# HuiGuanLab/Lite-MKD

Measured on AMD Instinct MI355X. Metric: episodes/sec (5-way 5-shot, 8x224^2 frames), higher is better.
Workload: dtype f32

## Files before the change

### lite-mkd_amd/csrc/conv.hip

```cpp
#include "gemm_core.h"
#include <atomic>
#include <mutex>

struct ConvGemmArgs {
  const float* src;
  const float* wpk;
  float* out;
  float* stat_partial;
  int N, Hs, Ws, Cs;
  int Hr, Wr, rows_per_class, tiles_per_class;
  int sh;
  int Ho, Wo, Co, omul;
  int Kp, cps, nclass;
  int n_rt, n_ct, xcd_mode;
  int taps_pm1;
  int grid_step;
  int grid_total;
  int same;
  int halo;
  int accum;
  const float* ep_stats;
  const float* ep_res;
  int ep_relu;
  const float* pre_stats;
// ... 1115 lines not shown
  return p.tiles_per_class;
}
extern "C" int lmkd_conv2d_fwd_row_tiles(int N, int H, int W, int Cout, int KH, int KW, int stride, int pad) {
  return lmkd_conv2d_fwd_row_tiles_cs(N, H, W, 32, Cout, KH, KW, stride, pad);
}

static int conv2d_fwd_impl(const float* x, const float* wp, float* y, float* stat_partial, const float* ep_stats,
                           const float* ep_res, int ep_relu, int N, int H, int W, int Cs, int Cout, int KH, int KW, int stride,
                           int pad, void* stream, const float* pre_stats = nullptr, int seg_n0 = 0, const lmkd_amax_desc* am = nullptr) {
  LMKD_REQUIRE(x && wp && y, "lmkd_conv2d_fwd: null pointer");
  if (seg_n0 <= 0 || seg_n0 >= N) seg_n0 = 0;
  LMKD_REQUIRE(!seg_n0 || (conv_planes() && !ep_stats), "lmkd_conv2d_fwd_seg: two frame segments exist in the bf16-plane modes (training / plain forward)");
  LMKD_REQUIRE(aligned16(x) && aligned16(wp), "lmkd_conv2d_fwd: x / packed weights must be 16-byte aligned");
  LMKD_REQUIRE(Cs % 32 == 0 || Cs == 4, "lmkd_conv2d_fwd: channel count %d must be 4 (padded stem) or a multiple of 32", Cs);
  LMKD_REQUIRE(N > 0 && H > 0 && W > 0 && Cout > 0, "lmkd_conv2d_fwd: empty tensor");
  const bool smallc = Cs == 4;
  const int KWp = kw_padded(Cs, KW);
  LMKD_REQUIRE(!smallc || KWp == 8, "lmkd_conv2d_fwd: padded-stem path needs KW <= 8");
  LMKD_REQUIRE(KH * (smallc ? 1 : KW) <= LMKD_MAX_TAPS, "lmkd_conv2d_fwd: kernel %dx%d has too many taps", KH, KW);
  LMKD_REQUIRE(H < 32768 && W < 32768, "lmkd_conv2d_fwd: spatial dims too large");
  const bool act16 = g_lmkd_act_bf16;
  LMKD_REQUIRE(!pre_stats || (stat_partial && !smallc && !act16),
               "lmkd_conv2d_fwd_pre: the fused BatchNorm+ReLU loader exists for the training forward with fp32 activations (stat_partial given, Cs %% 32 == 0)");
  LMKD_REQUIRE(!act16 || (conv_nprod() == 1 && !ep_stats), "bf16 activations need lmkd_conv_set_compute_dtype(1) (training / plain forward)");
  const int Ho = conv_out(H, KH, stride, pad), Wo = conv_out(W, KW, stride, pad);
  LMKD_REQUIRE(Ho > 0 && Wo > 0, "lmkd_conv2d_fwd: empty output");
  LMKD_REQUIRE((long)N * H * W * Cs < 2147483647L && (long)N * Ho * Wo * Cout < 2147483647L,
               "lmkd_conv2d_fwd: tensor exceeds 2^31 elements");
  LMKD_REQUIRE(!conv_planes() || (long)N * H * W * Cs * (act16 && Cs != 4 ? 2 : 4) < 0xffffffe0L,
               "lmkd_conv2d_fwd: input tensor exceeds the 4 GiB buffer range of the bf16-plane kernels");
  ConvGemmArgs a;
  fwd_geometry(a, N, H, W, Cs, Cout, KH, KW, stride, pad, seg_n0);
  a.src = x; a.wpk = wp; a.out = y; a.stat_partial = stat_partial;
  a.h2_xw = am ? (const unsigned*)am->x_words : nullptr;
  a.amax_out = am ? (unsigned*)am->out_words : nullptr;
  note_fenced(am);
  a.ep_stats = ep_stats; a.ep_res = ep_res; a.ep_relu = ep_relu;
  a.pre_stats = pre_stats;
  const ConvPlan p = plan_fwd(a, KH, KW, pad);
  if (p.src2) {
    LMKD_REQUIRE((long)N * H * W * Cs * 4 < 2147483647L, "lmkd_conv2d_fwd: input tensor exceeds the 2 GiB offset range of the stride-2 patch form");
    fwd_src2_args(a, W, KWp);
  }
  int rc = launch_conv(a, p, (hipStream_t)stream);
  if (rc == LMKD_OK && a.amax_out && p.amax_pass) {
    const long per = (long)Ho * Wo * Cout, n0 = seg_n0 ? seg_n0 * per : (long)N * per;
    rc = amax_impl(y, n0, a.amax_out, stream, false);
    if (rc == LMKD_OK && seg_n0) rc = amax_impl(y + n0, (long)N * per - n0, a.amax_out + LMKD_AMAX_SEG_WORDS, stream, false);
  }
  return rc;
}

extern "C" int lmkd_conv2d_fwd(const float* x, const float* wp, float* y, float* stat_partial, int N, int H, int W, int Cs,
                               int Cout, int KH, int KW, int stride, int pad, void* stream) {
  return conv2d_fwd_impl(x, wp, y, stat_partial, nullptr, nullptr, 0, N, H, W, Cs, Cout, KH, KW, stride, pad, stream);
}

extern "C" int lmkd_conv2d_fwd_seg(const float* x, const float* pre_stats, const float* wp, float* y, float* stat_partial, int N, int H, int W,
                                   int Cs, int Cout, int KH, int KW, int stride, int pad, int seg_n0, void* stream, const lmkd_amax_desc* amax) {
  return conv2d_fwd_impl(x, wp, y, stat_partial, nullptr, nullptr, 0, N, H, W, Cs, Cout, KH, KW, stride, pad, stream, pre_stats, seg_n0, amax);
}

extern "C" int lmkd_conv2d_fwd_pre(const float* x_raw, const float* pre_stats, const float* wp, float* y, float* stat_partial, int N,
                                   int H, int W, int Cs, int Cout, int KH, int KW, int stride, int pad, void* stream) {
  LMKD_REQUIRE(pre_stats, "lmkd_conv2d_fwd_pre: BatchNorm table of the input missing");
  return conv2d_fwd_impl(x_raw, wp, y, stat_partial, nullptr, nullptr, 0, N, H, W, Cs, Cout, KH, KW, stride, pad, stream, pre_stats);
}

extern "C" int lmkd_conv2d_fwd_bn(const float* x, const float* wp, float* y, const float* bn_stats, const float* res, int relu,
                                  int N, int H, int W, int Cs, int Cout, int KH, int KW, int stride, int pad, void* stream, const lmkd_amax_desc* amax) {
  LMKD_REQUIRE(bn_stats, "lmkd_conv2d_fwd_bn: BatchNorm table missing");
  LMKD_REQUIRE(!g_lmkd_act_bf16, "lmkd_conv2d_fwd_bn: fp32 tensors only (with bf16 tensors run lmkd_conv2d_fwd + lmkd_bn_apply)");
  LMKD_REQUIRE(!conv_planes() || Cs % 32 == 0, "lmkd_conv2d_fwd_bn: the bf16-plane modes need Cs %% 32 == 0 (Cs=%d)", Cs);
  return conv2d_fwd_impl(x, wp, y, nullptr, bn_stats, res, relu, N, H, W, Cs, Cout, KH, KW, stride, pad, stream, nullptr, 0, amax);
}

static int bwd_data_args(ConvGemmArgs& a, const float* dy, const float* wd, float* dx, int N, int H, int W, int Cin, int Cout, int KH, int KW,
                         int stride, int pad, int accumulate, int seg_n0 = 0, const lmkd_amax_desc* am = nullptr) {
  if (seg_n0 <= 0 || seg_n0 >= N) seg_n0 = 0;
  LMKD_REQUIRE(!seg_n0 || conv_planes(), "lmkd_conv2d_bwd_data_seg: two frame segments exist in the bf16-plane modes");
  LMKD_REQUIRE(Cout % 32 == 0, "lmkd_conv2d_bwd_data: Cout=%d must be a multiple of 32", Cout);
  LMKD_REQUIRE(stride == 1 || stride == 2, "lmkd_conv2d_bwd_data: stride %d unsupported", stride);
  LMKD_REQUIRE(KH * KW <= LMKD_MAX_TAPS, "lmkd_conv2d_bwd_data: kernel too large");
  LMKD_REQUIRE(!g_lmkd_act_bf16 || conv_nprod() == 1, "bf16 activations need lmkd_conv_set_compute_dtype(1)");
  const int Ho = conv_out(H, KH, stride, pad), Wo = conv_out(W, KW, stride, pad);
  LMKD_REQUIRE((long)N * H * W * Cin < 2147483647L && (long)N * Ho * Wo * Cout < 2147483647L,
               "lmkd_conv2d_bwd_data: tensor exceeds 2^31 elements");
  LMKD_REQUIRE(!conv_planes() || (long)N * Ho * Wo * Cout * (g_lmkd_act_bf16 ? 2 : 4) < 0xffffffe0L,
               "lmkd_conv2d_bwd_data: dy exceeds the 4 GiB buffer range of the bf16-plane kernels");
  dgrad_geometry(a, N, H, W, Cin, Cout, KH, KW, stride, pad, seg_n0);
  a.src = dy; a.wpk = wd; a.out = dx; a.accum = accumulate;
  a.h2_xw = am ? (const unsigned*)am->dy_words : nullptr;
  return LMKD_OK;
}

extern "C" int lmkd_conv2d_bwd_data(const float* dy, const float* wd, float* dx, int N, int H, int W, int Cin, int Cout,
                                    int KH, int KW, int stride, int pad, int accumulate, void* stream) {
  LMKD_REQUIRE(dy && wd && dx, "lmkd_conv2d_bwd_data: null pointer");
  LMKD_REQUIRE(aligned16(dy) && aligned16(wd), "lmkd_conv2d_bwd_data: operands must be 16-byte aligned");
  ConvGemmArgs a;
  if (const int rc = bwd_data_args(a, dy, wd, dx, N, H, W, Cin, Cout, KH, KW, stride, pad, accumulate)) return rc;
  return launch_conv(a, plan_dgrad(a), (hipStream_t)stream);
}

extern "C" int lmkd_conv2d_bwd_data_bn_tiles_seg(int N, int H, int W, int Cin, int Cout, int KH, int KW, int stride, int pad, int seg_n0, int* tiles0) {
  if (stride != 1 || Cout % 32 != 0 || KH * KW > LMKD_MAX_TAPS) return 0;
  ConvGemmArgs a;
  if (bwd_data_args(a, nullptr, nullptr, nullptr, N, H, W, Cin, Cout, KH, KW, stride, pad, 0, seg_n0)) return 0;
  const ConvPlan p = plan_dgrad(a);
  if (!p.bnb_form) return 0;
  if (tiles0) *tiles0 = p.seg_t0;
  return p.tiles_per_class;
}
extern "C" int lmkd_conv2d_bwd_data_bn_tiles(int N, int H, int W, int Cin, int Cout, int KH, int KW, int stride, int pad) {
  return lmkd_conv2d_bwd_data_bn_tiles_seg(N, H, W, Cin, Cout, KH, KW, stride, pad, 0, nullptr);
}
extern "C" int lmkd_conv2d_bwd_data_seg(const float* dy, const float* wd, float* dx, const float* bn_x, const float* bn_stats, float* part, int N,
                                        int H, int W, int Cin, int Cout, int KH, int KW, int stride, int pad, int accumulate, int seg_n0, void* stream,
                                        const lmkd_amax_desc* amax) {
  LMKD_REQUIRE(dy && wd && dx, "lmkd_conv2d_bwd_data_seg: null pointer");
  LMKD_REQUIRE(aligned16(dy) && aligned16(wd), "lmkd_conv2d_bwd_data_seg: operands must be 16-byte aligned");
  LMKD_REQUIRE((bn_x != nullptr) == (bn_stats != nullptr) && (bn_x != nullptr) == (part != nullptr), "lmkd_conv2d_bwd_data_seg: bn_x, bn_stats and part go together");
  ConvGemmArgs a;
  if (const int rc = bwd_data_args(a, dy, wd, dx, N, H, W, Cin, Cout, KH, KW, stride, pad, accumulate, seg_n0, amax)) return rc;
  note_fenced(amax);
  if (bn_x) {
    LMKD_REQUIRE(!accumulate && aligned16(bn_x) && aligned16(bn_stats), "lmkd_conv2d_bwd_data_seg: the fused BatchNorm sums need a plain (non-accumulating) launch and aligned operands");
    a.bnb_x = bn_x; a.bnb_stats = bn_stats; a.stat_partial = part;
  }
  const ConvPlan p = plan_dgrad(a);
  LMKD_REQUIRE(!bn_x || p.bnb_form, "lmkd_conv2d_bwd_data_seg: this launch has no fused form (lmkd_conv2d_bwd_data_bn_tiles_seg returned 0)");
  return launch_conv(a, p, (hipStream_t)stream);
}
extern "C" int lmkd_conv2d_bwd_data_bn(const float* dy, const float* wd, float* dx, const float* bn_x, const float* bn_stats, float* part,
                                       int N, int H, int W, int Cin, int Cout, int KH, int KW, int stride, int pad, void* stream) {
  LMKD_REQUIRE(dy && wd && dx && bn_x && bn_stats && part, "lmkd_conv2d_bwd_data_bn: null pointer");
  LMKD_REQUIRE(aligned16(dy) && aligned16(wd) && aligned16(bn_x) && aligned16(bn_stats), "lmkd_conv2d_bwd_data_bn: operands must be 16-byte aligned");
  ConvGemmArgs a;
  if (const int rc = bwd_data_args(a, dy, wd, dx, N, H, W, Cin, Cout, KH, KW, stride, pad, 0)) return rc;
  a.bnb_x = bn_x; a.bnb_stats = bn_stats; a.stat_partial = part;
  const ConvPlan p = plan_dgrad(a);
  LMKD_REQUIRE(p.bnb_form, "lmkd_conv2d_bwd_data_bn: this launch has no fused form (lmkd_conv2d_bwd_data_bn_tiles returned 0)");
  return launch_conv(a, p, (hipStream_t)stream);
}

static int g_wgrad_planes = 1;
extern "C" int lmkd_conv_set_wgrad_planes(int on) { g_wgrad_planes = on ? 1 : 0; return LMKD_OK; }
static int g_wgrad_win16 = 1;
extern "C" int lmkd_conv_set_wgrad_win16(int on) { g_wgrad_win16 = on ? 1 : 0; return LMKD_OK; }
static int g_wgrad_window = 1;
extern "C" int lmkd_conv_set_wgrad_window(int on) { g_wgrad_window = on < 0 ? 0 : on; return LMKD_OK; }
static inline bool wgrad_win_eligible(int W, int Cs, int Cout, int KH, int KW, int stride, int pad) {
  return g_wgrad_window && g_wgrad_planes && conv_planes() && KH == 3 && KW == 3 && stride == 1 && pad == 1 &&
         Cs % 32 == 0 && 32 + 2 * (W + 1) <= 256;
}
static void wgrad_win_plan(int Mpix, int W, int Cs, int Cout, int* cob, int* splits, int* steps_per_split) {
  *cob = Cout >= 128 ? 4 : 2;
  const int tiles = cdiv(Cout, 32 * *cob) * (Cs / 32);
  const int steps = cdiv(Mpix, LMKD_BK);
  const int warm = cdiv(2 * (W + 1), LMKD_BK);
  const int resident = 256 * ((conv_nprod() >= 6 && *cob == 2) ? 2 : 8 / *cob);
  int sp = g_wgrad_window > 1 ? cdiv(g_wgrad_window, tiles)
                              : std::max((int)(((long)resident * steps + 19600L * 4 / *cob) / (39200L * 4 / *cob)), cdiv(128, tiles));
  const int cap = std::max(1, steps / (12 * warm));
  if (sp > cap) sp = cap;
  *steps_per_split = cdiv(steps, sp);
  *splits = cdiv(steps, *steps_per_split);
}

static void wgrad_plan(int Mpix, int Cout, int Kp, int* splits, int* steps_per_split, int* bm, int* bn, bool planes = false) {
  *bm = Cout <= 64 ? 64 : 128;
  *bn = (Kp % 128 == 0 && Kp >= 1024) ? 128 : 64;
  int per_cu = (*bm == 128 && *bn == 128) ? 2 : ((*bm == 64 && *bn == 64) ? 4 : 3);
  if (planes) {
    if (*bm == 64 && *bn == 128) *bn = 64;
    const int npl = conv_nprod() == 1 ? 1 : 3;
    const long lds = 1L * npl * LMKD_BK * ((*bm * 2 + 64) + (*bn * 2 + 64));
    per_cu = (int)(160 * 1024 / lds);
    if (per_cu > 4) per_cu = 4;
    if (per_cu < 1) per_cu = 1;
  }
  const int tiles = cdiv(Cout, *bm) * cdiv(Kp, *bn);
  const int steps = cdiv(Mpix, LMKD_BK);
  const int slots = 256 * per_cu;
  int best_sp = 1;
  double best_cost = 1e30;
  for (int r = 1; r <= 3; ++r) {
    int sp = (slots * r) / tiles;
    if (sp > steps / 4) sp = steps / 4;
    if (sp < 1) sp = 1;
    const int sps = cdiv(steps, sp);
    sp = cdiv(steps, sps);
    const double rounds = (double)cdiv((long)tiles * sp, slots);
    const double cost = rounds * sps + 1.0 * sp / 8.0;
    if (cost < best_cost) { best_cost = cost; best_sp = sp; }
  }
  if (planes && *bm == 64 && *bn == 64 && best_sp < cdiv(steps, 64)) best_sp = cdiv(steps, 64);
  *steps_per_split = cdiv(steps, best_sp);
  *splits = cdiv(steps, *steps_per_split);
}

static int g_wgrad_stem = 1;
extern "C" int lmkd_conv_set_wgrad_stem(int on) { g_wgrad_stem = on ? 1 : 0; return LMKD_OK; }
static int stem_wgrad_plan(int N, int H, int W, int Cs, int Cout, int KH, int KW, int stride, int pad, int* G) {
  if (!g_wgrad_stem || !g_wgrad_planes || conv_nprod(g_lmkd_act_bf16) < 6 || Cs != 4 || Cout != 64 || KH != 7 || KW != 7 || stride != 2 || pad != 3) return 0;
  const int Ho = conv_out(H, KH, stride, pad), Wo = conv_out(W, KW, stride, pad);
  if (Wo < 17 || Wo > 128 || W > 2 * Wo || Ho < 1) return 0;
  const int units = N * cdiv(Ho, 2);
  int g = std::max(1, 2048 / (2 * Wo));
  g = std::min(g, std::max(1, units / 256));
  *G = g;
  return cdiv(units, g);
}

enum class WgFam : unsigned char {
  Stem,
  Win16,
  Win,
  Planes,
  Tile,
};
struct WgradPlan {
  WgFam fam;
  bool pre, act16, smallc;
  int nprod;
  int bm, bn;
  int cob;
  int G;
  int splits, splits0, sps0, sps1, seg_pix0;
  int xcd;
  int grid;
  long need;
  long ws;
};

static long wgrad_workspace(int N, int H, int W, int Cs, int Cout, int KH, int KW, int stride, int pad) {
  const int Ho = conv_out(H, KH, stride, pad), Wo = conv_out(W, KW, stride, pad);
  const int Kp = KH * kw_padded(Cs, KW) * Cs;
  int G, splits, sps, bm, bn;
  if (const int slabs = stem_wgrad_plan(N, H, W, Cs, Cout, KH, KW, stride, pad, &G)) return (long)slabs * Cout * Kp * sizeof(float);
  wgrad_plan(N * Ho * Wo, Cout, Kp, &splits, &sps, &bm, &bn, conv_planes() && g_wgrad_planes);
  if (wgrad_win_eligible(W, Cs, Cout, KH, KW, stride, pad)) {
    int cob, wsplits, wsps;
    wgrad_win_plan(N * Ho * Wo, W, Cs, Cout, &cob, &wsplits, &wsps);
    splits = std::max(splits, wsplits);
  }
  return (long)splits * Cout * Kp * sizeof(float);
}

static WgradPlan plan_wgrad(int N, int H, int W, int Cs, int Cout, int KH, int KW, int stride, int pad, int seg_n0, bool pre, bool maxima) {
  WgradPlan p;
  memset(&p, 0, sizeof(p));
  const bool act16 = g_lmkd_act_bf16;
  const int Ho = conv_out(H, KH, stride, pad), Wo = conv_out(W, KW, stride, pad);
  const int Kp = KH * kw_padded(Cs, KW) * Cs, Mpix = N * Ho * Wo;
  p.pre = pre; p.act16 = act16; p.smallc = Cs == 4;
  p.ws = wgrad_workspace(N, H, W, Cs, Cout, KH, KW, stride, pad);
  if (seg_n0)
    p.ws = std::max(p.ws, wgrad_workspace(seg_n0, H, W, Cs, Cout, KH, KW, stride, pad) + wgrad_workspace(N - seg_n0, H, W, Cs, Cout, KH, KW, stride, pad));
  p.seg_pix0 = seg_n0 ? seg_n0 * Ho * Wo : Mpix;
  if (const int slabs = stem_wgrad_plan(N, H, W, Cs, Cout, KH, KW, stride, pad, &p.G)) {
    p.fam = WgFam::Stem;
    p.nprod = conv_nprod(false, maxima);
    p.splits = p.grid = slabs;
  } else if (wgrad_win_eligible(W, Cs, Cout, KH, KW, stride, pad)) {
    const bool w16 = g_wgrad_win16 && conv_nprod(act16) >= 6;
    p.fam = w16 ? WgFam::Win16 : WgFam::Win;
    p.nprod = w16 ? conv_nprod(false, maxima) : conv_nprod(act16);
    wgrad_win_plan(Mpix, W, Cs, Cout, &p.cob, &p.splits, &p.sps0);
    p.splits0 = p.splits;
    if (seg_n0) {
      int sp1, cob1;
      wgrad_win_plan(p.seg_pix0, W, Cs, Cout, &p.cob, &p.splits0, &p.sps0);
      wgrad_win_plan(Mpix - p.seg_pix0, W, Cs, Cout, &cob1, &sp1, &p.sps1);
      p.splits = p.splits0 + sp1;
    }
    p.grid = 8 * cdiv(p.splits, 8) * cdiv(Cout, 32 * p.cob) * (Cs / 32);
  } else {
    const bool planes = conv_planes() && g_wgrad_planes;
    p.fam = planes ? WgFam::Planes : WgFam::Tile;
    p.nprod = planes ? conv_nprod(act16, maxima && !p.smallc && !pre) : (conv_nprod() == 1 ? 1 : 0);
    wgrad_plan(Mpix, Cout, Kp, &p.splits, &p.sps0, &p.bm, &p.bn, planes);
    p.splits0 = p.splits;
    if (seg_n0) {
      int sp1, bm1, bn1;
      wgrad_plan(p.seg_pix0, Cout, Kp, &p.splits0, &p.sps0, &p.bm, &p.bn, planes);
      wgrad_plan(Mpix - p.seg_pix0, Cout, Kp, &sp1, &p.sps1, &bm1, &bn1, planes);
      p.splits = p.splits0 + sp1;
    }
    p.xcd = (g_xcd_mode != 0 && g_xcd_mode != 1 && p.splits >= 32) ? 1 : 0;
    p.grid = (p.xcd ? 8 * cdiv(p.splits, 8) : p.splits) * cdiv(Cout, p.bm) * cdiv(Kp, p.bn);
  }
  p.need = (long)p.splits * Cout * Kp * sizeof(float);
  return p;
}

template <int NPROD, int D, int RLC>
static void launch_stem_wgrad(const StemWgradArgs& w, dim3 grid, size_t lds, hipStream_t s) {
  lds_attr_once<stem_wgrad_kernel<NPROD, D, RLC>>(160 * 1024);
  hipLaunchKernelGGL((stem_wgrad_kernel<NPROD, D, RLC>), grid, dim3(512), lds, s, w);
}
template <int NPROD>
static void launch_stem_wgrad(const StemWgradArgs& w, dim3 grid, size_t lds, hipStream_t s) {
  const bool deep = cdiv(2 * w.Wo, 32) >= 6;
  if (deep && w.RL == 1856) launch_stem_wgrad<NPROD, 6, 1856>(w, grid, lds, s);
  else if (deep) launch_stem_wgrad<NPROD, 6, 0>(w, grid, lds, s);
  else launch_stem_wgrad<NPROD, 2, 0>(w, grid, lds, s);
}
template <int COB>
static void launch_wgrad_win(const WgradWinArgs& w, const WgradPlan& p, bool big, hipStream_t s) {
  const dim3 grid(p.grid);
  if (p.fam == WgFam::Win16) {
    constexpr int JW = COB == 2 ? 1 : 2;
    constexpr int NT = 64 * COB * (2 / JW);
    with_nprod<3, 6, 9>(p.nprod, [&](auto np) {
      if (big && p.pre) hipLaunchKernelGGL((conv_wgrad_win16_kernel<COB, np, 256, true, 9, JW>), grid, dim3(NT), 0, s, w);
      else if (big) hipLaunchKernelGGL((conv_wgrad_win16_kernel<COB, np, 256, false, 9, JW>), grid, dim3(NT), 0, s, w);
      else if (p.pre) hipLaunchKernelGGL((conv_wgrad_win16_kernel<COB, np, 128, true, 9, JW>), grid, dim3(NT), 0, s, w);
      else hipLaunchKernelGGL((conv_wgrad_win16_kernel<COB, np, 128, false, 9, JW>), grid, dim3(NT), 0, s, w);
    });
    return;
  }
  auto go = [&](auto np, auto a16, auto pre) {
    constexpr int NPROD = decltype(np)::value;
    constexpr bool A16 = decltype(a16)::value, PRE = decltype(pre)::value;
    constexpr int TPW = (COB == 2 && NPROD != 1) ? 5 : 9;
    constexpr int NT = 64 * COB * ((9 + TPW - 1) / TPW);
    if (big) hipLaunchKernelGGL((conv_wgrad_win_kernel<COB, NPROD, A16, 256, PRE, TPW>), grid, dim3(NT), 0, s, w);
    else hipLaunchKernelGGL((conv_wgrad_win_kernel<COB, NPROD, A16, 128, PRE, TPW>), grid, dim3(NT), 0, s, w);
  };
  using T = std::true_type;
  using F = std::false_type;
  if (p.act16) go(std::integral_constant<int, 1>{}, T{}, F{});
  else with_nprod<1, 6, 9>(p.nprod, [&](auto np) { if (p.pre) go(np, F{}, T{}); else go(np, F{}, F{}); });
}

template <class CFG>
static void launch_wgrad_planes(const WgradArgs& a, const WgradPlan& p, hipStream_t s) {
  const dim3 grid(p.grid), block(256);
  if (p.act16) {
    if (p.smallc) hipLaunchKernelGGL((conv_wgrad_x3_kernel<CFG, true, 1, false, true>), grid, block, 0, s, a);
    else hipLaunchKernelGGL((conv_wgrad_x3_kernel<CFG, false, 1, false, true>), grid, block, 0, s, a);
  } else if (p.smallc) {
    with_nprod<1, 6, 9>(p.nprod, [&](auto np) { hipLaunchKernelGGL((conv_wgrad_x3_kernel<CFG, true, np, false>), grid, block, 0, s, a); });
  } else if (p.pre) {
    with_nprod<1, 6, 9>(p.nprod, [&](auto np) { hipLaunchKernelGGL((conv_wgrad_x3_kernel<CFG, false, np, true>), grid, block, 0, s, a); });
  } else {
    with_nprod<1, 3, 6, 9>(p.nprod, [&](auto np) { hipLaunchKernelGGL((conv_wgrad_x3_kernel<CFG, false, np, false>), grid, block, 0, s, a); });
  }
}

template <class CFG, bool SM, int THR>
static void launch_wgrad_tile(const WgradArgs& a, const WgradPlan& p, hipStream_t s) {
  const dim3 grid(p.grid);
  if (p.nprod == 1) hipLaunchKernelGGL((conv_wgrad_kernel<CFG, SM, true>), grid, dim3(THR), 0, s, a);
  else if (!SM && p.pre) hipLaunchKernelGGL((conv_wgrad_kernel<CFG, false, false, true>), grid, dim3(THR), 0, s, a);
  else hipLaunchKernelGGL((conv_wgrad_kernel<CFG, SM, false>), grid, dim3(THR), 0, s, a);
}

static int conv2d_bwd_weight_impl(const float* x, const float* pre_stats, const float* dy, float* dw_oihw, float* workspace,
                                  long ws_bytes, int N, int H, int W, int Cs, int Cin, int Cout, int KH, int KW, int stride, int pad,
                                  void* stream, int accumulate = 0, int seg_n0 = 0, const lmkd_amax_desc* am = nullptr) {
  const unsigned* amax_x = am ? (const unsigned*)am->x_words : nullptr;
  const unsigned* amax_dy = am ? (const unsigned*)am->dy_words : nullptr;
  note_fenced(am);
  LMKD_REQUIRE(x && dy && dw_oihw && workspace, "lmkd_conv2d_bwd_weight: null pointer");
  if (seg_n0 <= 0 || seg_n0 >= N) seg_n0 = 0;
  LMKD_REQUIRE(aligned16(x) && aligned16(dy) && aligned16(workspace), "lmkd_conv2d_bwd_weight: operands must be 16-byte aligned");
  LMKD_REQUIRE(Cs % 32 == 0 || Cs == 4, "lmkd_conv2d_bwd_weight: channel count %d must be 4 or a multiple of 32", Cs);
  LMKD_REQUIRE(Cout % 4 == 0, "lmkd_conv2d_bwd_weight: Cout %% 4 != 0");
  const bool smallc = Cs == 4;
  const WgradPlan p = plan_wgrad(N, H, W, Cs, Cout, KH, KW, stride, pad, seg_n0, pre_stats != nullptr, amax_x && amax_dy);
  LMKD_REQUIRE(!seg_n0 || p.fam != WgFam::Tile, "lmkd_conv2d_bwd_weight_seg: two frame segments exist in the bf16-plane modes");
  LMKD_REQUIRE(!pre_stats || (!smallc && (conv_nprod() != 1 || p.fam != WgFam::Tile) && !p.act16), "lmkd_conv2d_bwd_weight_pre: Cs %% 32 == 0, fp32 activations only");
  LMKD_REQUIRE(!p.act16 || (conv_nprod() == 1 && p.fam != WgFam::Tile), "bf16 activations need lmkd_conv_set_compute_dtype(1) and the plane weight-gradient kernel");
  const int Ho = conv_out(H, KH, stride, pad), Wo = conv_out(W, KW, stride, pad);
  const int KWp = kw_padded(Cs, KW), Kp = KH * KWp * Cs, Mpix = N * Ho * Wo;
  LMKD_REQUIRE((long)N * H * W * Cs < 2147483647L && (long)Mpix * Cout < 2147483647L, "lmkd_conv2d_bwd_weight: tensor too large");
  LMKD_REQUIRE(ws_bytes >= p.need, "lmkd_conv2d_bwd_weight: workspace too small");
  hipStream_t s = (hipStream_t)stream;
  if (p.fam == WgFam::Stem) {
    LMKD_REQUIRE((long)Mpix * 64 * 4 < 0xffffffe0L && (long)N * H * W * 16 < 0xffffffe0L, "lmkd_conv2d_bwd_weight: tensor too large for 32-bit byte offsets");
    StemWgradArgs w;
    memset(&w, 0, sizeof(w));
    w.dy = dy; w.x = x; w.slab = workspace;
    w.h2_xw = amax_x; w.h2_dyw = amax_dy;
    w.N = N; w.H = H; w.W = W; w.Ho = Ho; w.Wo = Wo;
    w.upi = cdiv(Ho, 2); w.units = N * w.upi; w.G = p.G; w.slabs = p.splits;
    w.RL = 16 * Wo + 64;
    const size_t lds = (size_t)2 * 10 * 3 * w.RL + 2 * 3 * STEM_WG_APLANE;
    with_nprod<3, 6, 9>(p.nprod, [&](auto np) { launch_stem_wgrad<np>(w, dim3(p.grid), lds, s); });
    LMKD_CHECK_LAUNCH("stem_wgrad_kernel");
    if (Kp <= 256) {
      hipLaunchKernelGGL(wgrad_reduce_stem_kernel, dim3(Cout), dim3(256, 4), 0, s, (const float*)workspace, dw_oihw, p.splits, Cout, Cin, Cs, KH, KW,
                         KWp, Kp, accumulate);
    } else {
      launch_wgrad_reduce((const float*)workspace, dw_oihw, p.splits, Cout, Cin, Cs, KH, KW, KWp, Kp, accumulate, s);
    }
    LMKD_CHECK_LAUNCH("wgrad_reduce_kernel");
    return LMKD_OK;
  }
  if (p.fam == WgFam::Win16 || p.fam == WgFam::Win) {
    LMKD_REQUIRE((long)Mpix * std::max(Cs, Cout) * 4 < 2147483647L, "lmkd_conv2d_bwd_weight: tensor too large for 32-bit byte offsets");
    WgradWinArgs w;
    memset(&w, 0, sizeof(w));
    w.dy = dy; w.x = x; w.slab = workspace; w.pre_stats = pre_stats;
    w.h2_xw = amax_x; w.h2_dyw = amax_dy;
    w.N = N; w.H = H; w.W = W; w.Cs = Cs; w.Co = Cout; w.Kp = Kp; w.Mpix = Mpix;
    w.steps_total = cdiv(Mpix, LMKD_BK);
    w.splits = p.splits; w.steps_per_split = p.sps0;
    w.seg_pix0 = p.seg_pix0; w.seg_splits0 = p.splits0; w.sps1 = p.sps1;
    w.n_ct = cdiv(Cout, 32 * p.cob); w.n_it = Cs / 32;
    w.div_hw = make_fastdiv(H * W); w.div_w = make_fastdiv(W);
    const bool big = 32 + 2 * (W + 1) > 128;
    if (p.cob == 4) launch_wgrad_win<4>(w, p, big, s);
    else launch_wgrad_win<2>(w, p, big, s);
    LMKD_CHECK_LAUNCH("conv_wgrad_win_kernel");
    launch_wgrad_reduce((const float*)workspace, dw_oihw, p.splits, Cout, Cin, Cs, KH, KW, KWp, Kp, accumulate, s);
    LMKD_CHECK_LAUNCH("wgrad_reduce_kernel");
    return LMKD_OK;
  }
  WgradArgs a;
  memset(&a, 0, sizeof(a));
  a.dy = dy; a.x = x; a.slab = workspace; a.pre_stats = pre_stats;
  a.h2_xw = amax_x; a.h2_dyw = amax_dy;
  a.N = N; a.Hs = H; a.Ws = W; a.Cs = Cs;
  a.Ho = Ho; a.Wo = Wo; a.Co = Cout;
  a.stride = stride; a.pad = pad; a.KH = KH; a.KW = KW; a.KWp = KWp;
  a.Kp = Kp; a.Mpix = Mpix;
  a.steps_per_split = p.sps0;
  a.seg_pix0 = p.seg_pix0; a.seg_splits0 = p.splits0; a.sps1 = p.sps1;
  a.steps_total = cdiv(Mpix, LMKD_BK);
  a.div_hw = make_fastdiv(Ho * Wo); a.div_w = make_fastdiv(Wo);
  a.n_mt = cdiv(Cout, p.bm); a.n_jt = cdiv(Kp, p.bn); a.splits = p.splits;
  a.xcd_mode = p.xcd;
  const int bm = p.bm, bn = p.bn;
  LMKD_REQUIRE(!smallc || (bm == 64 && bn == 64), "lmkd_conv2d_bwd_weight: padded-stem path expects Cout <= 64");
  if (p.fam == WgFam::Planes) {
    if (bm == 128 && bn == 128) launch_wgrad_planes<WgCfg<128, 128, 2, 2>>(a, p, s);
    else if (bm == 128) launch_wgrad_planes<WgCfg<128, 64, 2, 2>>(a, p, s);
    else launch_wgrad_planes<WgCfg<64, 64, 2, 2>>(a, p, s);
    LMKD_CHECK_LAUNCH("conv_wgrad_x3_kernel");
  } else {
    if (smallc) launch_wgrad_tile<TileCfg<64, 64, 2, 2>, true, LMKD_THREADS>(a, p, s);
    else if (bm == 64 && bn == 64) launch_wgrad_tile<TileCfg<64, 64, 2, 2>, false, LMKD_THREADS>(a, p, s);
    else if (bm == 128 && bn == 64) launch_wgrad_tile<TileCfg<128, 64, 2, 2>, false, LMKD_THREADS>(a, p, s);
    else if (bm == 64 && bn == 128) launch_wgrad_tile<TileCfg<64, 128, 2, 2>, false, LMKD_THREADS>(a, p, s);
    else launch_wgrad_tile<TileCfg<128, 128, 2, 4>, false, 512>(a, p, s);
    LMKD_CHECK_LAUNCH("conv_wgrad_kernel");
  }
  launch_wgrad_reduce((const float*)workspace, dw_oihw, p.splits, Cout, Cin, Cs, KH, KW, KWp, Kp, accumulate, s);
  LMKD_CHECK_LAUNCH("wgrad_reduce_kernel");
  return LMKD_OK;
}

extern "C" long lmkd_conv2d_bwd_weight_workspace_seg(int N, int H, int W, int Cs, int Cout, int KH, int KW, int stride, int pad, int seg_n0) {
  if (seg_n0 <= 0 || seg_n0 >= N) seg_n0 = 0;
  return plan_wgrad(N, H, W, Cs, Cout, KH, KW, stride, pad, seg_n0, false, false).ws;
}
extern "C" long lmkd_conv2d_bwd_weight_workspace(int N, int H, int W, int Cs, int Cout, int KH, int KW, int stride, int pad) {
  return lmkd_conv2d_bwd_weight_workspace_seg(N, H, W, Cs, Cout, KH, KW, stride, pad, 0);
}

extern "C" int lmkd_conv2d_bwd_weight(const float* x, const float* dy, float* dw_oihw, float* workspace, long ws_bytes,
                                      int N, int H, int W, int Cs, int Cin, int Cout, int KH, int KW, int stride, int pad,
                                      void* stream) {
  return conv2d_bwd_weight_impl(x, nullptr, dy, dw_oihw, workspace, ws_bytes, N, H, W, Cs, Cin, Cout, KH, KW, stride, pad, stream);
}

extern "C" int lmkd_conv2d_bwd_weight_pre(const float* x_raw, const float* pre_stats, const float* dy, float* dw_oihw,
                                          float* workspace, long ws_bytes, int N, int H, int W, int Cs, int Cin, int Cout, int KH,
                                          int KW, int stride, int pad, void* stream) {
  LMKD_REQUIRE(pre_stats, "lmkd_conv2d_bwd_weight_pre: BatchNorm table of the input missing");
  return conv2d_bwd_weight_impl(x_raw, pre_stats, dy, dw_oihw, workspace, ws_bytes, N, H, W, Cs, Cin, Cout, KH, KW, stride, pad, stream);
}

extern "C" int lmkd_conv2d_bwd_weight_acc(const float* x, const float* pre_stats, const float* dy, float* dw_oihw, float* workspace,
                                          long ws_bytes, int N, int H, int W, int Cs, int Cin, int Cout, int KH, int KW, int stride,
                                          int pad, void* stream) {
  return conv2d_bwd_weight_impl(x, pre_stats, dy, dw_oihw, workspace, ws_bytes, N, H, W, Cs, Cin, Cout, KH, KW, stride, pad, stream, 1);
}


extern "C" int lmkd_conv2d_bwd_weight_seg(const float* x, const float* pre_stats, const float* dy, float* dw_oihw, float* workspace, long ws_bytes,
                                          int N, int H, int W, int Cs, int Cin, int Cout, int KH, int KW, int stride, int pad, int accumulate,
                                          int seg_n0, void* stream, const lmkd_amax_desc* amax) {
  return conv2d_bwd_weight_impl(x, pre_stats, dy, dw_oihw, workspace, ws_bytes, N, H, W, Cs, Cin, Cout, KH, KW, stride, pad, stream, accumulate, seg_n0, amax);
}

extern "C" int lmkd_conv2d_plan(int kind, int N, int H, int W, int Cs, int Cin, int Cout, int KH, int KW, int stride, int pad,
                                int* info) {
  LMKD_REQUIRE(info && kind >= 0 && kind <= 2, "lmkd_conv2d_plan: kind must be 0 (forward), 1 (data gradient) or 2 (weight gradient)");
  LMKD_REQUIRE(N > 0 && H > 0 && W > 0 && Cout > 0 && KH > 0 && KW > 0 && stride > 0, "lmkd_conv2d_plan: bad shape");
  if (kind == 2) {
    const WgradPlan p = plan_wgrad(N, H, W, Cs, Cout, KH, KW, stride, pad, 0, false, false);
    info[1] = p.xcd; info[2] = p.splits; info[3] = p.grid;
    switch (p.fam) {
      case WgFam::Stem: info[0] = 14; info[4] = 2; break;
      case WgFam::Win16:
      case WgFam::Win: info[0] = p.cob == 4 ? 5 : 6; info[1] = 1; info[4] = 1; break;
      default: info[0] = (p.bm == 128 && p.bn == 128) ? 1 : (p.bm == 128 ? 2 : (p.bn == 128 ? 4 : 3)); info[4] = 0; break;
    }
    return LMKD_OK;
  }
  ConvGemmArgs a;
  if (kind == 0) fwd_geometry(a, N, H, W, Cs, Cout, KH, KW, stride, pad, 0);
  else dgrad_geometry(a, N, H, W, Cin, Cout, KH, KW, stride, pad, 0);
  const ConvPlan p = kind == 0 ? plan_fwd(a, KH, KW, pad) : plan_dgrad(a);
  info[0] = p.tile; info[1] = p.xcd; info[2] = p.nclass; info[3] = p.grid;
  info[4] = p.fam == ConvFam::Stem ? 2 : (p.fam == ConvFam::Patch || p.fam == ConvFam::Patch16 || p.fam == ConvFam::Patch1p ? 1 : 0);
  return LMKD_OK;
}
```

### lite-mkd_amd/csrc/wgrad_stem.h

```cpp
#pragma once

struct StemWgradArgs {
  const float* dy;
  const float* x;
  float* slab;
  int N, H, W, Ho, Wo;
  int upi;
  int units, G, slabs;
  int RL;
  const unsigned* h2_xw;
  const unsigned* h2_dyw;
};

#define STEM_WG_LDA 160
#define STEM_WG_APLANE (32 * STEM_WG_LDA)

template <int V> struct StemSlot { static constexpr int value = V; };

template <int NPROD, int D, int RLC>
__global__ __launch_bounds__(512) void stem_wgrad_kernel(StemWgradArgs a) {
  static_assert(NPROD == 6 || NPROD == 9 || NPROD == 3, "three bf16 planes (6 / 9 products) or two fp16 planes (3 products: conv_patch16.h)");
  constexpr int NPL = NPROD == 3 ? 2 : 3;
  extern __shared__ __attribute__((aligned(16))) unsigned char smem[];
  const int RL = RLC ? RLC : a.RL;
  const int XBUF = 10 * NPL * RL;
  unsigned char* s_x = smem;
  unsigned char* s_dy = smem + 2 * XBUF;
  const int tid = threadIdx.x, lane = tid & 63, wave = tid >> 6;
  const int cb = wave & 3, nb = wave >> 2;
  const int q4 = lane >> 4, idx = lane & 15;
  const int W = a.W, Wo = a.Wo;

  for (int i = tid; i < (2 * XBUF) / 16; i += 512) reinterpret_cast<u32x4*>(s_x)[i] = u32x4{0u, 0u, 0u, 0u};

  const __amdgpu_buffer_rsrc_t rs_dy = x3_rsrc(a.dy, (long)a.N * a.Ho * Wo * 64 * 4);
  const __amdgpu_buffer_rsrc_t rs_x = x3_rsrc(a.x, (long)a.N * a.H * W * 4 * 4);

  float h2_sx = 1.f, h2_sdy = 1.f;
  if constexpr (NPROD == 3) {
    const unsigned mx0 = amax_read(a.h2_xw, 0), mx1 = amax_read(a.h2_xw, 1), md0 = amax_read(a.h2_dyw, 0), md1 = amax_read(a.h2_dyw, 1);
    h2_sx = h2_scale(mx0 > mx1 ? mx0 : mx1);
    h2_sdy = h2_scale(md0 > md1 ? md0 : md1);
  }
  const int d_k = tid >> 4, d_c = (tid & 15) * 4;
  u32x4 rq[D];
  u32x4 rx[9];
  auto as_f4 = [](const u32x4& r) { return make_float4(__uint_as_float(r.x), __uint_as_float(r.y), __uint_as_float(r.z), __uint_as_float(r.w)); };
  struct Pos { int u, ks, n, oh0, limit; };
  const int ksteps = (2 * Wo + 31) >> 5;
  auto set_unit = [&](Pos& p, int u) {
    p.u = u;
    p.ks = 0;
    if (u < 0) return;
    p.n = u / a.upi;
    p.oh0 = 2 * (u - p.n * a.upi);
    p.limit = (a.Ho - p.oh0 >= 2 ? 2 : 1) * Wo;
  };
  auto next_unit = [&](int u) {
    const int s = u / a.G;
    if (u + 1 < a.units && (u + 1) / a.G == s) return u + 1;
    const long ns = (long)s + gridDim.x;
    return ns < a.slabs ? (int)(ns * a.G) : -1;
  };
  auto load_dy = [&](u32x4& r, const Pos& p) {
    const int k = 32 * p.ks + d_k;
    r = __builtin_amdgcn_raw_buffer_load_b128(rs_dy, k < p.limit ? (unsigned)((((p.n * a.Ho + p.oh0) * Wo + k) * 64 + d_c) * 4) : X3_OOB, 0, 0);
  };
  auto load_x = [&](const Pos& p) {
#pragma unroll
    for (int j = 0; j < 9; ++j) {
      const int ih = 2 * p.oh0 - 3 + j;
      rx[j] = __builtin_amdgcn_raw_buffer_load_b128(rs_x, (tid < W && (unsigned)ih < (unsigned)a.H) ? (unsigned)((((p.n * a.H + ih) * W + tid) * 4) * 4) : X3_OOB, 0, 0);
    }
  };
  auto store_x = [&](int buf) {
    if (tid >= W) return;
    unsigned char* d = s_x + buf * XBUF + (tid + 3) * 8;
#pragma unroll
    for (int j = 0; j < 9; ++j) {
      uint2 p0, p1, p2;
      if constexpr (NPROD == 3) h2_split4(as_f4(rx[j]), h2_sx, p0, p1); else x3_split4(as_f4(rx[j]), p0, p1, p2);
      *reinterpret_cast<uint2*>(d + (j * NPL + 0) * RL) = p0;
      *reinterpret_cast<uint2*>(d + (j * NPL + 1) * RL) = p1;
      if constexpr (NPL == 3) *reinterpret_cast<uint2*>(d + (j * NPL + 2) * RL) = p2;
    }
  };

  const int a_off = (4 * q4 + (idx >> 2)) * STEM_WG_LDA + (16 * cb + 4 * (idx & 3)) * 2;
  const int b_col = 32 * nb + 8 * (idx & 3);
  f32x4 acc[7];
#pragma unroll
  for (int kh = 0; kh < 7; ++kh) acc[kh] = f32x4{0.f, 0.f, 0.f, 0.f};
  if ((int)blockIdx.x >= a.slabs) return;
  Pos cp, pf;
  set_unit(cp, (int)blockIdx.x * a.G);
  pf = cp;
  bool x_pending = false;
  auto advance_pf = [&]() {
    if (++pf.ks < ksteps) return;
    set_unit(pf, next_unit(pf.u));
    if (pf.u >= 0) {
      load_x(pf);
      x_pending = true;
    }
  };
  __syncthreads();
  load_x(cp);
  store_x(0);
#pragma unroll
  for (int d = 0; d < D; ++d) {
    if (pf.u >= 0) {
      load_dy(rq[d], pf);
      advance_pf();
    }
  }
  int xb = 0;
  int gstep = 0;
  auto step = [&](auto slot) {
    constexpr int S = decltype(slot)::value;
    if constexpr (NPROD == 3) tr_store4_h2<STEM_WG_LDA, STEM_WG_APLANE>(s_dy + (gstep & 1) * NPL * STEM_WG_APLANE, d_k, d_c, as_f4(rq[S]), h2_sdy);
    else tr_store4<NPL, STEM_WG_LDA, STEM_WG_APLANE>(s_dy + (gstep & 1) * NPL * STEM_WG_APLANE, d_k, d_c, as_f4(rq[S]));
    if (x_pending && cp.ks == ksteps - 1) {
      store_x(xb ^ 1);
      x_pending = false;
    }
    __syncthreads();
    if (pf.u >= 0) {
      load_dy(rq[S], pf);
      advance_pf();
    }
    const unsigned char* dyb = s_dy + (gstep & 1) * NPL * STEM_WG_APLANE;
    unsigned badr[2];
#pragma unroll
    for (int hh = 0; hh < 2; ++hh) {
      const int k = 32 * cp.ks + 16 * hh + 4 * q4 + (idx >> 2);
      const int r = k >= Wo ? 1 : 0;
      badr[hh] = (unsigned)(xb * XBUF + b_col + 2 * r * NPL * RL + 16 * (k - r * Wo));
    }
    bf16x8 fa[NPL];
#pragma unroll
    for (int p = 0; p < NPL; ++p) {
      const s16x4_t lo = __builtin_amdgcn_ds_read_tr16_b64_v4i16((s16x4_t __attribute__((address_space(3)))*)(dyb + p * STEM_WG_APLANE + a_off));
      const s16x4_t hi = __builtin_amdgcn_ds_read_tr16_b64_v4i16((s16x4_t __attribute__((address_space(3)))*)(dyb + p * STEM_WG_APLANE + a_off + 16 * STEM_WG_LDA));
      union { s16x4_t s[2]; bf16x8 b; } uu;
      uu.s[0] = lo; uu.s[1] = hi;
      fa[p] = uu.b;
    }
    bf16x8 fb[2][NPL];
    auto read_b = [&](int kh, bf16x8 (&f)[NPL]) {
#pragma unroll
      for (int p = 0; p < NPL; ++p) {
        const s16x4_t lo = __builtin_amdgcn_ds_read_tr16_b64_v4i16((s16x4_t __attribute__((address_space(3)))*)(s_x + badr[0] + (kh * NPL + p) * RL));
        const s16x4_t hi = __builtin_amdgcn_ds_read_tr16_b64_v4i16((s16x4_t __attribute__((address_space(3)))*)(s_x + badr[1] + (kh * NPL + p) * RL));
        union { s16x4_t s[2]; bf16x8 b; } uu;
        uu.s[0] = lo; uu.s[1] = hi;
        f[p] = uu.b;
      }
    };
    read_b(0, fb[0]);
#pragma unroll
    for (int kh = 0; kh < 7; ++kh) {
      if (kh + 1 < 7) read_b(kh + 1, fb[(kh + 1) & 1]);
      __builtin_amdgcn_sched_barrier(0);
      const bf16x8(&b)[NPL] = fb[kh & 1];
      f32x4 c = acc[kh];
      if constexpr (NPROD == 3) {
        c = __builtin_amdgcn_mfma_f32_16x16x32_f16(__builtin_bit_cast(f16x8, fa[1]), __builtin_bit_cast(f16x8, b[0]), c, 0, 0, 0);
        c = __builtin_amdgcn_mfma_f32_16x16x32_f16(__builtin_bit_cast(f16x8, fa[0]), __builtin_bit_cast(f16x8, b[1]), c, 0, 0, 0);
        c = __builtin_amdgcn_mfma_f32_16x16x32_f16(__builtin_bit_cast(f16x8, fa[0]), __builtin_bit_cast(f16x8, b[0]), c, 0, 0, 0);
      } else {
        if (NPROD == 9) {
          c = __builtin_amdgcn_mfma_f32_16x16x32_bf16(fa[NPL - 1], b[NPL - 1], c, 0, 0, 0);
          c = __builtin_amdgcn_mfma_f32_16x16x32_bf16(fa[1], b[NPL - 1], c, 0, 0, 0);
          c = __builtin_amdgcn_mfma_f32_16x16x32_bf16(fa[NPL - 1], b[1], c, 0, 0, 0);
        }
        c = __builtin_amdgcn_mfma_f32_16x16x32_bf16(fa[1], b[1], c, 0, 0, 0);
        c = __builtin_amdgcn_mfma_f32_16x16x32_bf16(fa[0], b[NPL - 1], c, 0, 0, 0);
        c = __builtin_amdgcn_mfma_f32_16x16x32_bf16(fa[NPL - 1], b[0], c, 0, 0, 0);
        c = __builtin_amdgcn_mfma_f32_16x16x32_bf16(fa[0], b[1], c, 0, 0, 0);
        c = __builtin_amdgcn_mfma_f32_16x16x32_bf16(fa[1], b[0], c, 0, 0, 0);
        c = __builtin_amdgcn_mfma_f32_16x16x32_bf16(fa[0], b[0], c, 0, 0, 0);
      }
      acc[kh] = c;
      __builtin_amdgcn_sched_barrier(0);
    }
    ++gstep;
    if (++cp.ks < ksteps) return;
    const int slab = cp.u / a.G;
    const int un = next_unit(cp.u);
    if (un < 0 || un / a.G != slab) {
      float* C = a.slab + (long)slab * 64 * 224;
#pragma unroll
      for (int kh = 0; kh < 7; ++kh) {
#pragma unroll
        for (int e = 0; e < 4; ++e)
          C[(16 * cb + 4 * q4 + e) * 224 + kh * 32 + 16 * nb + idx] = NPROD == 3 ? acc[kh][e] * (1.f / h2_sx) * (1.f / h2_sdy) : acc[kh][e];
        acc[kh] = f32x4{0.f, 0.f, 0.f, 0.f};
      }
    }
    set_unit(cp, un);
    xb ^= 1;
  };
  while (true) {
    step(StemSlot<0>());
    if (cp.u < 0) break;
    if constexpr (D > 1) {
      step(StemSlot<1>());
      if (cp.u < 0) break;
    }
    if constexpr (D > 2) {
      step(StemSlot<2>());
      if (cp.u < 0) break;
    }
    if constexpr (D > 3) {
      step(StemSlot<3>());
      if (cp.u < 0) break;
    }
    if constexpr (D > 4) {
      step(StemSlot<4>());
      if (cp.u < 0) break;
    }
    if constexpr (D > 5) {
      step(StemSlot<5>());
      if (cp.u < 0) break;
    }
  }
}
```

Before: 51.08.

## Single-buffer stem wgrad input tile to raise occupancy in fp16 path

The stem weight-gradient kernel drops the double-buffered LDS input (x) tile in favour of a single buffer. The next unit's x is stored behind an extra block barrier at each unit boundary, with its global load issued one unit ahead. LDS sizing now follows the plane count, and the fp16 (3-product) variant gets a prefetch depth of 2 and a launch bound asking for 4 blocks per CU. The aim is to fit more blocks per CU so latency is hidden by occupancy, at the cost of a serializing barrier and a store at each unit switch.

After: 50.12. -1.9%, worse.

```diff
diff --git a/lite-mkd_amd/csrc/conv.hip b/lite-mkd_amd/csrc/conv.hip
--- a/lite-mkd_amd/csrc/conv.hip
+++ b/lite-mkd_amd/csrc/conv.hip
@@ -1441,9 +1441,10 @@
 }
 template <int NPROD>
 static void launch_stem_wgrad(const StemWgradArgs& w, dim3 grid, size_t lds, hipStream_t s) {
+  constexpr int DD = NPROD == 3 ? STEM_WG_D2 : 6;
   const bool deep = cdiv(2 * w.Wo, 32) >= 6;
-  if (deep && w.RL == 1856) launch_stem_wgrad<NPROD, 6, 1856>(w, grid, lds, s);
-  else if (deep) launch_stem_wgrad<NPROD, 6, 0>(w, grid, lds, s);
+  if (deep && w.RL == 1856) launch_stem_wgrad<NPROD, DD, 1856>(w, grid, lds, s);
+  else if (deep) launch_stem_wgrad<NPROD, DD, 0>(w, grid, lds, s);
   else launch_stem_wgrad<NPROD, 2, 0>(w, grid, lds, s);
 }
 template <int COB>
@@ -1527,7 +1528,8 @@
     w.N = N; w.H = H; w.W = W; w.Ho = Ho; w.Wo = Wo;
     w.upi = cdiv(Ho, 2); w.units = N * w.upi; w.G = p.G; w.slabs = p.splits;
     w.RL = 16 * Wo + 64;
-    const size_t lds = (size_t)2 * 10 * 3 * w.RL + 2 * 3 * STEM_WG_APLANE;
+    const int npl = p.nprod == 3 ? 2 : 3;
+    const size_t lds = (size_t)10 * npl * w.RL + 2 * npl * STEM_WG_APLANE;
     with_nprod<3, 6, 9>(p.nprod, [&](auto np) { launch_stem_wgrad<np>(w, dim3(p.grid), lds, s); });
     LMKD_CHECK_LAUNCH("stem_wgrad_kernel");
     if (Kp <= 256) {
diff --git a/lite-mkd_amd/csrc/wgrad_stem.h b/lite-mkd_amd/csrc/wgrad_stem.h
--- a/lite-mkd_amd/csrc/wgrad_stem.h
+++ b/lite-mkd_amd/csrc/wgrad_stem.h
@@ -17,21 +17,22 @@
 
 template <int V> struct StemSlot { static constexpr int value = V; };
 
+#define STEM_WG_D2 2
 template <int NPROD, int D, int RLC>
-__global__ __launch_bounds__(512) void stem_wgrad_kernel(StemWgradArgs a) {
+__global__ __launch_bounds__(512, NPROD == 3 ? 4 : 2) void stem_wgrad_kernel(StemWgradArgs a) {
   static_assert(NPROD == 6 || NPROD == 9 || NPROD == 3, "three bf16 planes (6 / 9 products) or two fp16 planes (3 products: conv_patch16.h)");
   constexpr int NPL = NPROD == 3 ? 2 : 3;
   extern __shared__ __attribute__((aligned(16))) unsigned char smem[];
   const int RL = RLC ? RLC : a.RL;
   const int XBUF = 10 * NPL * RL;
   unsigned char* s_x = smem;
-  unsigned char* s_dy = smem + 2 * XBUF;
+  unsigned char* s_dy = smem + XBUF;
   const int tid = threadIdx.x, lane = tid & 63, wave = tid >> 6;
   const int cb = wave & 3, nb = wave >> 2;
   const int q4 = lane >> 4, idx = lane & 15;
   const int W = a.W, Wo = a.Wo;
 
-  for (int i = tid; i < (2 * XBUF) / 16; i += 512) reinterpret_cast<u32x4*>(s_x)[i] = u32x4{0u, 0u, 0u, 0u};
+  for (int i = tid; i < XBUF / 16; i += 512) reinterpret_cast<u32x4*>(s_x)[i] = u32x4{0u, 0u, 0u, 0u};
 
   const __amdgpu_buffer_rsrc_t rs_dy = x3_rsrc(a.dy, (long)a.N * a.Ho * Wo * 64 * 4);
   const __amdgpu_buffer_rsrc_t rs_x = x3_rsrc(a.x, (long)a.N * a.H * W * 4 * 4);
@@ -73,9 +74,9 @@
       rx[j] = __builtin_amdgcn_raw_buffer_load_b128(rs_x, (tid < W && (unsigned)ih < (unsigned)a.H) ? (unsigned)((((p.n * a.H + ih) * W + tid) * 4) * 4) : X3_OOB, 0, 0);
     }
   };
-  auto store_x = [&](int buf) {
+  auto store_x = [&]() {
     if (tid >= W) return;
-    unsigned char* d = s_x + buf * XBUF + (tid + 3) * 8;
+    unsigned char* d = s_x + (tid + 3) * 8;
 #pragma unroll
     for (int j = 0; j < 9; ++j) {
       uint2 p0, p1, p2;
@@ -92,21 +93,17 @@
 #pragma unroll
   for (int kh = 0; kh < 7; ++kh) acc[kh] = f32x4{0.f, 0.f, 0.f, 0.f};
   if ((int)blockIdx.x >= a.slabs) return;
-  Pos cp, pf;
+  Pos cp, pf, nx;
   set_unit(cp, (int)blockIdx.x * a.G);
   pf = cp;
-  bool x_pending = false;
   auto advance_pf = [&]() {
-    if (++pf.ks < ksteps) return;
-    set_unit(pf, next_unit(pf.u));
-    if (pf.u >= 0) {
-      load_x(pf);
-      x_pending = true;
-    }
+    if (++pf.ks == ksteps) set_unit(pf, next_unit(pf.u));
   };
   __syncthreads();
   load_x(cp);
-  store_x(0);
+  store_x();
+  set_unit(nx, next_unit(cp.u));
+  if (nx.u >= 0) load_x(nx);
 #pragma unroll
   for (int d = 0; d < D; ++d) {
     if (pf.u >= 0) {
@@ -114,16 +111,11 @@
       advance_pf();
     }
   }
-  int xb = 0;
   int gstep = 0;
   auto step = [&](auto slot) {
     constexpr int S = decltype(slot)::value;
     if constexpr (NPROD == 3) tr_store4_h2<STEM_WG_LDA, STEM_WG_APLANE>(s_dy + (gstep & 1) * NPL * STEM_WG_APLANE, d_k, d_c, as_f4(rq[S]), h2_sdy);
     else tr_store4<NPL, STEM_WG_LDA, STEM_WG_APLANE>(s_dy + (gstep & 1) * NPL * STEM_WG_APLANE, d_k, d_c, as_f4(rq[S]));
-    if (x_pending && cp.ks == ksteps - 1) {
-      store_x(xb ^ 1);
-      x_pending = false;
-    }
     __syncthreads();
     if (pf.u >= 0) {
       load_dy(rq[S], pf);
@@ -135,7 +127,7 @@
     for (int hh = 0; hh < 2; ++hh) {
       const int k = 32 * cp.ks + 16 * hh + 4 * q4 + (idx >> 2);
       const int r = k >= Wo ? 1 : 0;
-      badr[hh] = (unsigned)(xb * XBUF + b_col + 2 * r * NPL * RL + 16 * (k - r * Wo));
+      badr[hh] = (unsigned)(b_col + 2 * r * NPL * RL + 16 * (k - r * Wo));
     }
     bf16x8 fa[NPL];
 #pragma unroll
@@ -199,7 +191,11 @@
       }
     }
     set_unit(cp, un);
-    xb ^= 1;
+    if (un < 0) return;
+    __syncthreads();
+    store_x();
+    set_unit(nx, next_unit(un));
+    if (nx.u >= 0) load_x(nx);
   };
   while (true) {
     step(StemSlot<0>());
```
